# vandenheuvel/relp

Measured on AMD Instinct MI355X. Metric: simplex pivots/sec + wall-clock to optimal, Netlib 25fv47 @1 GPU, higher is better.
Workload: dtype f64; 1 GPU; Netlib 25FV47 821x1876, steepest-edge pricing, explicit-inverse carry, exact certificate inside the timed step, no presolve (+520 virtual artificials); carry=explicit, refactors=0, parallelism=1 LP per GPU x1, certified=True, objective_bits=1791

## Files before the change

### relp_amd/csrc/kernels.hip

```cpp
#include <hip/hip_runtime.h>
#include <hip/hip_ext.h>

#include <cmath>
#include <cstdlib>
#include <string>
#include <utility>

#include "kernels.hpp"
#include "pivot_step.hpp"
#include "price_step.hpp"
#include "solver.hpp"
#include "wave_ops.hpp"

namespace relp {


__global__ void budget_kernel(Ctl* ctl, long long add) {
    if (ctl->status == ST_BUDGET) ctl->status = ST_RUNNING;
    ctl->budget = ctl->iters + add;
}

typedef double f64x2_t __attribute__((ext_vector_type(2)));
template <int RULE, bool USE_LDS, int LPC, bool UNIT = false>
__global__ void __launch_bounds__(256) price_kernel(DeviceLP lp, int skip_weights, double tol_dual, int col_first,
                                                    int col_last, int cand_offset) {
    static_assert(!UNIT || LPC == 2, "generated columns are incidence columns");
    extern __shared__ __attribute__((aligned(16))) double smem[];
    __shared__ Cand s_cand[8];
    static_assert(LPC == ELL_W || LPC == 2, "one lane per padded entry (width 2 when no column has more than two entries: graph LPs)");
    constexpr int CPB = 256 / LPC;
    Ctl* ctl = lp.ctl;
    const int m = lp.m;
    const int g = threadIdx.x / LPC, sub = threadIdx.x % LPC;
    const int status = ctl->status;
    const int pending = (RULE == RELP_PIVOT_STEEPEST_EDGE) ? (ctl->pending && !skip_weights) : 0;
    const double gamma_q = ctl->gamma_q;
    const double alpha_pq = ctl->alpha_pq;
    const int leaving = ctl->leaving;
    const int last = ctl->last_selected;
    int base = col_first + blockIdx.x * CPB;
    int a = 0, b = 0, r0 = 0;
    double v0 = 0.0, cost_j = 0.0, g_j = 1.0;
    bool nonbasic = false;
    double sgn_j = 1.0;
    auto load_column = [&](int j) {
        a = b = r0 = 0;
        v0 = cost_j = 0.0;
        g_j = 1.0;
        nonbasic = false;
        sgn_j = 1.0;
        if (j < col_last) {
            const int pos_j = lp.pos[j];
            nonbasic = column_priced(pos_j);
            sgn_j = column_sign(pos_j);
            if (LPC != 2) {
                a = lp.col_start[j];
                b = lp.col_start[j + 1];
            }
            if (UNIT) {
                const unsigned code = (unsigned)lp.ell_rows[(size_t)j * LPC + sub];
                const bool absent = code == 0x7fffffffu;
                r0 = absent ? 0 : (int)(code & 0x7fffffffu);
                v0 = absent ? 0.0 : ((code >> 31) ? -1.0 : 1.0);
                cost_j = (double)lp.cost8[j];
            } else {
                r0 = lp.ell_rows[(size_t)j * LPC + sub];
                v0 = lp.ell_vals[(size_t)j * LPC + sub];
                cost_j = lp.cost[j];
            }
            if (RULE == RELP_PIVOT_STEEPEST_EDGE && !UNIT) g_j = lp.gamma[j];
        }
    };
    load_column(base + g);
    const double* v_pi = lp.minus_pi;
    const double* v_rho = lp.rho;
    const double* v_w = lp.w;
    if (USE_LDS) {
        double* s_pi = smem;
        double* s_rho = smem + m;
        double* s_w = smem + 2 * m;
        for (int i0 = threadIdx.x; i0 < m; i0 += 4 * 256) {
            double t_pi[4], t_rho[4], t_w[4];
#pragma unroll
            for (int u = 0; u < 4; ++u) {
                const int i = i0 + u * 256;
                t_pi[u] = i < m ? lp.minus_pi[i] : 0.0;
                t_rho[u] = i < m ? lp.rho[i] : 0.0;
                t_w[u] = i < m ? lp.w[i] : 0.0;
            }
#pragma unroll
            for (int u = 0; u < 4; ++u) {
                const int i = i0 + u * 256;
                if (i < m) {
                    s_pi[i] = t_pi[u];
                    s_rho[i] = t_rho[u];
                    s_w[i] = t_w[u];
                }
            }
        }
        v_pi = s_pi;
        v_rho = s_rho;
        v_w = s_w;
    }
    if (status != ST_RUNNING) return;
    if (USE_LDS) __syncthreads();

    Cand best = no_candidate();
    double best_cbar = 0.0;
    int best_row = 0, best_len = 0;
    double best_val = 0.0;
    while (base < col_last) {
        const int j = base + g;
        if (!nonbasic) { b = a; v0 = 0.0; }
        double d_pi, d_rho = 0.0, d_w = 0.0;
        if (UNIT) {
            d_pi = v0 * lp.minus_pi[r0];
            if (pending) {
                int hit = lp.rho_nz[r0] != 0 && v0 != 0.0;
                hit |= __shfl_xor(hit, 1);
                if (hit) {
                    d_rho = v0 * lp.rho[r0];
                    d_w = v0 * lp.w[r0];
                }
            }
        } else if (LPC == 2) {
            const double* t = lp.prw + (size_t)4 * r0;
            if (pending) {
                const f64x2_t lo = *reinterpret_cast<const f64x2_t*>(t);
                d_w = v0 * t[2];
                d_pi = v0 * lo.x;
                d_rho = v0 * lo.y;
            } else {
                d_pi = v0 * t[0];
            }
        } else {
            d_pi = v0 * v_pi[r0];
            if (pending) {
                d_rho = v0 * v_rho[r0];
                d_w = v0 * v_w[r0];
            }
        }
        for (int e = a + LPC + sub; e < b; e += LPC) {
            const int r = lp.row_index[e];
            const double v = lp.value[e];
            d_pi += v * v_pi[r];
            if (pending) {
                d_rho += v * v_rho[r];
                d_w += v * v_w[r];
            }
        }
        d_pi += dpp_f64<DPP_QUAD_1032, 0xF>(0.0, d_pi);
        if (LPC > 2) {
            d_pi += dpp_f64<DPP_QUAD_2301, 0xF>(0.0, d_pi);
            d_pi += dpp_f64<DPP_ROW_HALF_MIRROR, 0xF>(0.0, d_pi);
        }
        if (RULE == RELP_PIVOT_STEEPEST_EDGE) {
            d_rho += dpp_f64<DPP_QUAD_1032, 0xF>(0.0, d_rho);
            d_w += dpp_f64<DPP_QUAD_1032, 0xF>(0.0, d_w);
            if (LPC > 2) {
                d_rho += dpp_f64<DPP_QUAD_2301, 0xF>(0.0, d_rho);
                d_rho += dpp_f64<DPP_ROW_HALF_MIRROR, 0xF>(0.0, d_rho);
                d_w += dpp_f64<DPP_QUAD_2301, 0xF>(0.0, d_w);
                d_w += dpp_f64<DPP_ROW_HALF_MIRROR, 0xF>(0.0, d_w);
            }
        }
        int improved = 0;
        const double cbar = sgn_j * (cost_j + d_pi);
        const bool weight_changes = RULE == RELP_PIVOT_STEEPEST_EDGE && pending && (!UNIT || j == leaving || d_rho != 0.0);
        if (sub == 0 && nonbasic && (!UNIT || weight_changes || cbar < -tol_dual)) {
            double gam = g_j;
            if (UNIT && RULE == RELP_PIVOT_STEEPEST_EDGE) gam = lp.gamma[j];
            if (weight_changes) lp.gamma[j] = gam = weight_after_pivot(gam, d_rho, d_w, gamma_q, alpha_pq, j == leaving);
            bool candidate;
            const double key = price_key<RULE>(cbar, tol_dual, gam, j, last, lp.n, candidate);
            if (candidate && offer_candidate<RULE>(best, key, j)) {
                best_cbar = cbar;
                improved = 1;
            }
        }
        improved = __shfl(improved, threadIdx.x & (WAVE - 1) & ~(LPC - 1));
        if (improved) {
            best_row = r0;
            best_val = v0;
            best_len = LPC == 2 ? 2 : b - a;
        }
        base += gridDim.x * CPB;
        if (base < col_last) load_column(base + g);
    }
    const Cand blk = block_best_candidate<RULE>(best, s_cand);
    const int slot = cand_offset + blockIdx.x;
    int winner = (sub == 0 && blk.idx >= 0 && blk.idx == best.idx) ? 1 : 0;
    if (winner) publish_candidate(lp, slot, blk.key, blk.idx, best_cbar, best_len);
    winner = __shfl(winner, threadIdx.x & (WAVE - 1) & ~(LPC - 1));
    if (winner) publish_entry(lp, slot, sub, best_row, best_val);
    if (blk.idx < 0 && threadIdx.x == 0) publish_no_candidate(lp, slot);
}

template <int RULE>
__global__ void __launch_bounds__(256) price_unit_kernel(DeviceLP lp, int skip_weights, double tol_dual, int col_first,
                                                         int col_last, int cand_offset) {
    constexpr int U = PRICE_UNIT_ARCS;
    extern __shared__ __attribute__((aligned(16))) unsigned s_rho_bits[];
    __shared__ Cand s_cand[8];
    Ctl* ctl = lp.ctl;
#ifdef RELP_STAMPS
    unsigned long long t_prev__ = wall_clock64();
    const int stamp_base__ = blockIdx.x == 0 ? 32 : (blockIdx.x == gridDim.x - 1 ? 40 : -1);
    if (threadIdx.x == 0 && blockIdx.x == 0) {
        lp.dbg[48] += 1;
        *(volatile unsigned long long*)(lp.dbg + 49) = t_prev__;
    }
#define USTAMP(k) do { asm volatile("s_waitcnt vmcnt(0) lgkmcnt(0)" ::: "memory"); if (threadIdx.x == 0 && stamp_base__ >= 0) { unsigned long long t__ = wall_clock64(); lp.dbg[stamp_base__ + (k)] += t__ - t_prev__; t_prev__ = t__; } } while (0)
#else
#define USTAMP(k) do {} while (0)
#endif
    const int status = ctl->status;
    const int pending = (RULE == RELP_PIVOT_STEEPEST_EDGE) ? (ctl->pending && !skip_weights) : 0;
    const double gamma_q = ctl->gamma_q;
    const double alpha_pq = ctl->alpha_pq;
    const int leaving = ctl->leaving;
    const int last = ctl->last_selected;
    const uint2* arcs = reinterpret_cast<const uint2*>(lp.ell_rows);
    unsigned ca[U], cb[U];
    int pos[U];
    double cost[U];
    auto load_arcs = [&](int base) {
#pragma unroll
        for (int u = 0; u < U; ++u) {
            const int j = base + u * 256 + threadIdx.x;
            ca[u] = cb[u] = 0x7fffffffu;
            pos[u] = 0;
            cost[u] = 0.0;
            if (j < col_last) {
                const uint2 c = arcs[j];
                ca[u] = c.x;
                cb[u] = c.y;
                pos[u] = lp.pos[j];
                cost[u] = (double)lp.cost8[j];
            }
        }
// ... 1475 lines not shown
    __shared__ double s_amount;
    if (threadIdx.x == 0) {
        const double cbar_q = ctl->cbar_q;
        int toggle = -1;
        double amount = 0.0;
        if (p < 0 && !flip) {
            ctl_unbounded(*ctl, q, 0);
        } else if (flip) {
            const double sgn_q = lp.flipped[q] ? -1.0 : 1.0;
            toggle = q;
            amount = ub_q * sgn_q;
            ctl_bound_flip(lp, *ctl, q, sgn_q, ub_q, cbar_q, ctl->minus_obj, ctl->iters);
            ctl->xp = ub_q;
        } else {
            const int leaving_flipped = bounded ? lp.flipped[leaving] : 0;
            if (step.leaves_at_upper) {
                toggle = leaving;
                amount = up_p * (leaving_flipped ? -1.0 : 1.0);
            }
            lp.basis[p] = q;
            push_touched(lp, *ctl, p);
            ctl_basis_change(lp, *ctl, bounded, q, p, leaving, leaving_flipped, step, ub_q, cbar_q, alpha_pq, ctl->gamma_q, total, ctl->minus_obj, ctl->iters);
            ctl->rho_buf ^= 1;
        }
        s_toggle = toggle;
        s_amount = amount;
    }
    __syncthreads();
    const int toggle = s_toggle;
    if (toggle >= 0) {
        const double amount = s_amount;
        for (int e = lp.col_start[toggle] + threadIdx.x; e < lp.col_start[toggle + 1]; e += blockDim.x)
            lp.rhs[lp.row_index[e]] -= amount * lp.value[e];
    }
}

constexpr int K2F_NW = K2F_THREADS / WAVE;
constexpr int K2F_INLINE_BLOCKS = 128;

struct K2fShared {
    double akey[K2F_NW];
    unsigned long long arank[K2F_NW];
    double red[K2F_NW + 2];
    double red2[K2F_NW + 2];
    double cbarv[K2F_MAX_BLOCKS];
    int crows[K2F_INLINE_BLOCKS * ELL_W];
    double cvals[K2F_INLINE_BLOCKS * ELL_W];
    int clen[K2F_INLINE_BLOCKS];
    int rows[K2_COL_CHUNK];
    double vals[K2_COL_CHUNK];
    double bcast[4];
    int ibcast[2];
};
template <int RULE>
__device__ __forceinline__ void k2f_candidates(const DeviceLP& lp, int n_price_blocks, K2fShared& sm, double& ckey, unsigned long long& crank) {
    const int tid = threadIdx.x;
    for (int b = tid; b < n_price_blocks; b += K2F_THREADS) {
        const int j = lp.cand_j[b];
        const double k = lp.cand_key[b];
        sm.cbarv[b] = lp.cand_cbar[b];
        offer_entering<RULE>(k, j, b, ckey, crank);
    }
    if (n_price_blocks <= K2F_INLINE_BLOCKS) {
        for (int e = tid; e < n_price_blocks * ELL_W; e += K2F_THREADS) {
            sm.crows[e] = lp.cand_rows[e];
            sm.cvals[e] = lp.cand_vals[e];
        }
        for (int b = tid; b < n_price_blocks; b += K2F_THREADS) sm.clen[b] = lp.cand_len[b];
    }
}
template <int RULE>
__device__ __forceinline__ int k2f_entering(double ckey, unsigned long long crank, K2fShared& sm, double& cbar_q, int& winner_block) {
    const int q = entering_winner<RULE>(ckey, crank, sm.akey, sm.arank, winner_block);
    cbar_q = q >= 0 ? sm.cbarv[winner_block] : 0.0;
    return q;
}
template <int R>
__device__ __forceinline__ void k2f_ftran_inline(const DeviceLP& lp, const double* T, const K2fShared& sm, int q, int winner_block,
                                                 double (&al)[R], int& ca, int& cb_) {
    const int tid = threadIdx.x, m = lp.m, ld = lp.ld;
    const int len = sm.clen[winner_block];
#pragma unroll
    for (int r = 0; r < R; ++r) {
        const int i = tid + r * K2F_THREADS;
        if (i >= m || len < 0) continue;
        const double* col = T + i;
        double t[ELL_W];
#pragma unroll
        for (int e = 0; e < ELL_W; ++e) t[e] = col[(size_t)sm.crows[winner_block * ELL_W + e] * ld];
        double a0 = 0.0;
#pragma unroll
        for (int e = 0; e < ELL_W; ++e) a0 += t[e] * sm.cvals[winner_block * ELL_W + e];
        al[r] = a0;
    }
    if (len > ELL_W || len < 0) {
        ca = lp.col_start[q] + (len < 0 ? 0 : ELL_W);
        cb_ = lp.col_start[q + 1];
    }
}
template <int R>
__device__ __forceinline__ void k2f_ftran_csc(const DeviceLP& lp, const double* T, K2fShared& sm, int ca, int cb_, double (&al)[R]) {
    const int tid = threadIdx.x, m = lp.m, ld = lp.ld;
    for (int c0 = ca; c0 < cb_; c0 += K2_COL_CHUNK) {
        const int cnt = min(K2_COL_CHUNK, cb_ - c0);
        __syncthreads();
        for (int e = tid; e < cnt; e += K2F_THREADS) {
            sm.rows[e] = lp.row_index[c0 + e];
            sm.vals[e] = lp.value[c0 + e];
        }
        __syncthreads();
        if constexpr (R <= 8) {
            double acc[R][4];
            int row[R];
#pragma unroll
            for (int r = 0; r < R; ++r) {
                const int i = tid + r * K2F_THREADS;
                row[r] = i < m ? i : 0;
                acc[r][0] = acc[r][1] = acc[r][2] = acc[r][3] = 0.0;
            }
            int e = 0;
            for (; e + 4 <= cnt; e += 4) {
                const size_t o0 = (size_t)sm.rows[e] * ld, o1 = (size_t)sm.rows[e + 1] * ld, o2 = (size_t)sm.rows[e + 2] * ld, o3 = (size_t)sm.rows[e + 3] * ld;
                const double v0 = sm.vals[e], v1 = sm.vals[e + 1], v2 = sm.vals[e + 2], v3 = sm.vals[e + 3];
                double x[R][4];
#pragma unroll
                for (int r = 0; r < R; ++r) {
                    x[r][0] = T[o0 + row[r]];
                    x[r][1] = T[o1 + row[r]];
                    x[r][2] = T[o2 + row[r]];
                    x[r][3] = T[o3 + row[r]];
                }
#pragma unroll
                for (int r = 0; r < R; ++r) {
                    acc[r][0] += x[r][0] * v0;
                    acc[r][1] += x[r][1] * v1;
                    acc[r][2] += x[r][2] * v2;
                    acc[r][3] += x[r][3] * v3;
                }
            }
            for (; e < cnt; ++e) {
                const size_t o = (size_t)sm.rows[e] * ld;
                const double v = sm.vals[e];
                double x[R];
#pragma unroll
                for (int r = 0; r < R; ++r) x[r] = T[o + row[r]];
#pragma unroll
// ... 50 lines not shown
    __syncthreads();
    if (wave == 0) {
        double t1 = lane < K2F_NW ? sm.red[lane] : 0.0;
        double t2 = lane < K2F_NW ? sm.red2[lane] : INFINITY;
        t1 = wave_sum(t1);
        t2 = wave_min(t2);
        if (lane == LAST) {
            sm.red[K2F_NW] = t1;
            sm.red2[K2F_NW] = t2;
        }
    }
    __syncthreads();
    gamma_q = 1.0 + sm.red[K2F_NW];
    theta_max = sm.red2[K2F_NW];
}
template <int R>
__device__ __forceinline__ int k2f_pass2(bool textbook, const double (&al)[R], const bool (&eligible)[R], const double (&room)[R],
                                         const int (&bas)[R], double theta_max, K2fShared& sm) {
    double hkey = 0.0;
    unsigned long long hrank = RANK_NONE;
#pragma unroll
    for (int r = 0; r < R; ++r) {
        const double mag = fabs(al[r]);
        if (eligible[r] && harris_accepts(room[r], mag, theta_max))
            keep_better(harris_key(textbook, mag), leaving_rank(bas[r], threadIdx.x + r * K2F_THREADS), hkey, hrank);
    }
    block_argbest(hkey, hrank, sm.akey, sm.arank);
    return leaving_row(hrank);
}
template <int R>
__device__ __forceinline__ void k2f_broadcast_row(int p, const double (&al)[R], const double (&xb)[R], const double (&room)[R],
                                                  const int (&bas)[R], K2fShared& sm) {
#pragma unroll
    for (int r = 0; r < R; ++r) {
        if ((int)threadIdx.x + r * K2F_THREADS == p) {
            sm.bcast[1] = al[r];
            sm.bcast[2] = xb[r];
            sm.bcast[3] = room[r];
            sm.ibcast[0] = bas[r];
        }
    }
    __syncthreads();
}

template <int RULE, int R>
__global__ void __launch_bounds__(K2F_THREADS) ftran_ratio_fast_kernel(DeviceLP lp, int n_price_blocks, double tol_pivot,
                                                                     double harris_delta, int skip_artificial_rows,
                                                                     int mode, int n_alpha_slices) {
    __shared__ K2fShared sm;
    Ctl* ctl = lp.ctl;
    STAMP_INIT;
    const int tid = threadIdx.x;
    const int m = lp.m;
    const int status = ctl->status;
    const long long iters = ctl->iters;
    const long long budget = ctl->budget;
    const int forced_q = ctl->forced_q;
    const int forced_p = ctl->forced_p;
    const double minus_obj = ctl->minus_obj;
    double xb[R];
    int bas[R];
#pragma unroll
    for (int r = 0; r < R; ++r) {
        const int i = tid + r * K2F_THREADS;
        xb[r] = i < m ? lp.xB[i] : 0.0;
        bas[r] = i < m ? lp.basis[i] : 0x7fffffff;
    }
    double ckey = 0.0;
    unsigned long long crank = RANK_NONE;
    const bool preselected = n_alpha_slices > 0;
    const int q_pre = preselected ? ctl->q : -1;
    const double cbar_pre = preselected ? ctl->cbar_q : 0.0;
    double ain[R];
#pragma unroll
    for (int r = 0; r < R; ++r) {
        const int i = tid + r * K2F_THREADS;
        ain[r] = (preselected && i < m) ? lp.alpha_in[i] : 0.0;
    }
    if (!preselected) k2f_candidates<RULE>(lp, n_price_blocks, sm, ckey, crank);
    const bool inline_column = forced_q < 0 && !preselected && n_price_blocks <= K2F_INLINE_BLOCKS;
    if (status != ST_RUNNING) return;
    STAMP(0);
    if (mode == 0 && iters >= budget) {
        if (tid == 0) ctl_budget(*ctl);
        return;
    }
    int q;
    double cbar_q;
    int winner_block = 0;
    if (preselected && forced_q < 0) {
        q = q_pre;
        cbar_q = cbar_pre;
    } else if (forced_q < 0) {
        q = k2f_entering<RULE>(ckey, crank, sm, cbar_q, winner_block);
    } else {
        q = forced_q;
        if (tid == 0) {
            double cb = lp.cost[forced_q];
            for (int e = lp.col_start[forced_q]; e < lp.col_start[forced_q + 1]; ++e) cb += lp.value[e] * lp.minus_pi[lp.row_index[e]];
            sm.bcast[0] = cb;
        }
        __syncthreads();
        cbar_q = sm.bcast[0];
        __syncthreads();
    }
    STAMP(1);
    if (q < 0) {
        if (tid == 0) ctl_no_entering(*ctl, mode);
        return;
    }
    if (mode == 1) {
        if (tid == 0) ctl_entering_only(*ctl, q, cbar_q);
        return;
    }
    double al[R];
#pragma unroll
    for (int r = 0; r < R; ++r) al[r] = 0.0;
    int ca = 0, cb_ = 0;
    if (inline_column) {
        k2f_ftran_inline<R>(lp, lp.Binv, sm, q, winner_block, al, ca, cb_);
    } else if (!preselected) {
        ca = lp.col_start[q];
        cb_ = lp.col_start[q + 1];
    }
    if (preselected) {
#pragma unroll
        for (int r = 0; r < R; ++r) al[r] += ain[r];
    }
    k2f_ftran_csc<R>(lp, lp.Binv, sm, ca, cb_, al);
    STAMP(2);
    const bool bounded = lp.ub != nullptr;
    double sgn_q = 1.0, ub_q = INFINITY;
// ... 102 lines not shown
        }
    }
    STAMP(5);
    const int leaving_flipped = bounded ? lp.flipped[leaving] : 0;
    if (step.leaves_at_upper) {
        const double sgn_l = leaving_flipped ? -1.0 : 1.0;
        for (int e = lp.col_start[leaving] + tid; e < lp.col_start[leaving + 1]; e += K2F_THREADS)
            lp.rhs[lp.row_index[e]] -= step.ub_leaving * sgn_l * lp.value[e];
    }
    if (bounded) __syncthreads();
    if (tid == 0) {
        lp.basis[p] = q;
        push_touched(lp, *ctl, p);
        if (lp.eta_cap > 0) {
            int is_new = 0;
            if (eta_slot_p < 0) {
                const int k = ctl->eta_count;
                lp.eta_slot[p] = k;
                lp.eta_rows[k] = p;
                ctl->eta_count = k + 1;
                is_new = 1;
            }
            ctl->eta_new = is_new;
            ctl->eta_version = ctl->eta_version + 1;
        }
        ctl_basis_change(lp, *ctl, bounded, q, p, leaving, leaving_flipped, step, ub_q, cbar_q, alpha_pq, gamma_q, total, minus_obj, iters);
        ctl->rho_buf ^= 1;
    }
    STAMP(6);
}

constexpr int KF_THREADS = K2F_THREADS;
constexpr int KF_NW = KF_THREADS / WAVE;
template <int RULE, int KF_R>
__global__ void __launch_bounds__(KF_THREADS) pivot_fused_kernel(DeviceLP lp, DeviceLP::State in, DeviceLP::State out, int n_price_blocks,
                                                                 double tol_pivot, double harris_delta, int skip_artificial_rows) {
    constexpr int R = KF_R;
    constexpr int KF_U = KF_R * KF_THREADS / WAVE;
    constexpr int KF_M = KF_R * KF_THREADS;
    __shared__ K2fShared sm;
    __shared__ double s_alpha[KF_M];
    const Ctl* ctl = in.ctl;
    const int tid = threadIdx.x;
    const int lane = tid & (WAVE - 1), wave = tid / WAVE;
#ifdef RELP_STAMPS
    unsigned long long t_prev__ = clock64();
    if (tid == 0 && blockIdx.x == 0) lp.dbg[63] += 1;
#define FSTAMP(k) do { if (tid == 0 && blockIdx.x == 0) { unsigned long long t__ = clock64(); lp.dbg[(k)] += t__ - t_prev__; t_prev__ = t__; } } while (0)
#else
#define FSTAMP(k) do {} while (0)
#endif
    const int m = lp.m, ld = lp.ld;
    const bool writer = blockIdx.x == 0;
    const int status = ctl->status;
    const long long iters = ctl->iters;
    const long long budget = ctl->budget;
    const double minus_obj = ctl->minus_obj;
    const int t_buf = ctl->t_buf;
    double xb[R];
    int bas[R];
#pragma unroll
    for (int r = 0; r < R; ++r) {
        const int i = tid + r * KF_THREADS;
        xb[r] = i < m ? in.xB[i] : 0.0;
        bas[r] = i < m ? in.basis[i] : 0x7fffffff;
    }
    double ckey = 0.0;
    unsigned long long crank = RANK_NONE;
    k2f_candidates<RULE>(lp, n_price_blocks, sm, ckey, crank);
    const bool inline_column = n_price_blocks <= K2F_INLINE_BLOCKS;
    auto hand_on = [&](auto verdict) {
        if (!writer) return;
#pragma unroll
        for (int r = 0; r < R; ++r) {
            const int i = tid + r * KF_THREADS;
            if (i < m) {
                out.xB[i] = xb[r];
                out.basis[i] = bas[r];
            }
        }
        if (tid == 0) {
            Ctl c = *ctl;
            verdict(c);
            c.forced_q = -1;
            c.forced_p = -1;
            *out.ctl = c;
        }
    };
    if (status != ST_RUNNING) {
        hand_on([](Ctl&) {});
        return;
    }
    FSTAMP(0);
    if (iters >= budget) {
        hand_on([](Ctl& c) { ctl_budget(c); });
        return;
    }
    double cbar_q;
    int winner_block = 0;
    const int q = k2f_entering<RULE>(ckey, crank, sm, cbar_q, winner_block);
    if (q < 0) {
        hand_on([](Ctl& c) { ctl_no_entering(c, 0); });
        return;
    }
    FSTAMP(1);
    const int j_own = blockIdx.x * KF_NW + wave;
    const bool own = j_own < m;
    const double* t_old = (t_buf ? lp.Binv2 : lp.Binv);
    double* t_new = (t_buf ? lp.Binv : lp.Binv2);
    const double* c_old = t_old + (size_t)(own ? j_own : 0) * ld;
    double o[KF_U];
#pragma unroll
    for (int u = 0; u < KF_U; ++u) {
        const int i = lane + u * WAVE;
        o[u] = (own && i < m) ? c_old[i] : 0.0;
    }
    const double pi_old = (own && lane == LAST) ? lp.minus_pi[j_own] : 0.0;
    double al[R];
#pragma unroll
    for (int r = 0; r < R; ++r) al[r] = 0.0;
    int ca = 0, cb_ = 0;
    if (inline_column) {
        k2f_ftran_inline<R>(lp, t_old, sm, q, winner_block, al, ca, cb_);
    } else {
        ca = lp.col_start[q];
        cb_ = lp.col_start[q + 1];
    }
    k2f_ftran_csc<R>(lp, t_old, sm, ca, cb_, al);
    FSTAMP(2);
    const HarrisRule harris = harris_rule(harris_delta);
    double sumsq = 0.0, theta = INFINITY;
    bool eligible[R];
    double room[R];
    k2f_pass1<R>(lp, false, al, xb, bas, tol_pivot, harris.slack, skip_artificial_rows, eligible, room, sumsq, theta);
#pragma unroll
    for (int r = 0; r < R; ++r) s_alpha[tid + r * KF_THREADS] = al[r];
    double gamma_q, theta_max;
    k2f_reduce(sm, sumsq, theta, gamma_q, theta_max);
    FSTAMP(3);
    const int p = k2f_pass2<R>(harris.textbook, al, eligible, room, bas, theta_max, sm);
    if (p < 0) {
        hand_on([q](Ctl& c) { ctl_unbounded(c, q, 0); });
        return;
    }
    FSTAMP(4);
    k2f_broadcast_row<R>(p, al, xb, room, bas, sm);
    const double alpha_pq = sm.bcast[1];
    const int leaving = sm.ibcast[0];
    const Step step = step_decision(false, false, p, alpha_pq, sm.bcast[2], sm.bcast[3], INFINITY);
    const double xp = step.xp;
    if (writer) {
#pragma unroll
        for (int r = 0; r < R; ++r) {
            const int i = tid + r * KF_THREADS;
            if (i < m) {
                lp.alpha[i] = al[r];
                out.xB[i] = (i == p) ? xp : xb[r] - al[r] * xp;
                out.basis[i] = (i == p) ? q : bas[r];
            }
        }
        if (tid == 0) {
            Ctl c = *ctl;
            ctl_basis_change(lp, c, false, q, p, leaving, 0, step, INFINITY, cbar_q, alpha_pq, gamma_q, 0, minus_obj, iters);
            c.t_buf = t_buf ^ 1;
            *out.ctl = c;
        }
    }
    FSTAMP(5);
    if (!own) return;
    const int u_p = p >> 6, lane_p = p & (WAVE - 1);
    double o_p = 0.0;
#pragma unroll
    for (int u = 0; u < KF_U; ++u) o_p = (u == u_p) ? o[u] : o_p;
    const double r_j = __shfl(o_p, lane_p) / alpha_pq;
    double* c_new = t_new + (size_t)j_own * ld;
    double w_j = 0.0;
#pragma unroll
    for (int u = 0; u < KF_U; ++u) {
        const int i = lane + u * WAVE;
        const double a = s_alpha[i];
        w_j += a * o[u];
        if (i < m) c_new[i] = (i == p) ? r_j : ((a != 0.0) ? o[u] - a * r_j : o[u]);
    }
    w_j = wave_sum(w_j);
    if (lane == LAST) {
        lp.w[j_own] = w_j;
        lp.rho[j_own] = r_j;
        lp.minus_pi[j_own] = pi_old - cbar_q * r_j;
    }
    FSTAMP(6);
}
#undef FSTAMP
__global__ void __launch_bounds__(256) begin_batch_kernel(DeviceLP lp, long long add) {
    const DeviceLP::State s0 = lp.state[0];
    for (int i = threadIdx.x; i < lp.m; i += 256) {
        s0.xB[i] = lp.xB[i];
        s0.basis[i] = lp.basis[i];
    }
    if (threadIdx.x == 0) {
        Ctl c = *lp.ctl;
        if (c.status == ST_BUDGET) c.status = ST_RUNNING;
        c.budget = c.iters + add;
        *lp.ctl = c;
        *s0.ctl = c;
    }
}
__global__ void __launch_bounds__(256) commit_kernel(DeviceLP lp, int parity) {
    const DeviceLP::State last = lp.state[parity];
    const int t_buf = last.ctl->t_buf;
    const int m = lp.m, ld = lp.ld;
    if (t_buf) {
        const int lane = threadIdx.x & (WAVE - 1);
        for (int j = blockIdx.x * 4 + threadIdx.x / WAVE; j < m; j += gridDim.x * 4) {
            const double* src = lp.Binv2 + (size_t)j * ld;
            double* dst = lp.Binv + (size_t)j * ld;
            for (int i = lane; i < m; i += WAVE) dst[i] = src[i];
        }
    }
    if (blockIdx.x == 0) {
        for (int i = threadIdx.x; i < m; i += 256) {
            lp.xB[i] = last.xB[i];
            lp.basis[i] = last.basis[i];
        }
        if (threadIdx.x == 0) {
            Ctl c = *last.ctl;
            c.t_buf = 0;
            *lp.ctl = c;
            if (lp.ctl_mirror) {
                *lp.ctl_mirror = c;
                __threadfence_system();
            }
        }
    }
// ... 830 lines not shown
```

### relp_amd/csrc/solver.hpp

```cpp
#pragma once
#include <cstdlib>
#include <cstring>
#include <cstddef>
#include <hip/hip_runtime.h>

#include <atomic>
#include <memory>
#include <mutex>
#include <stdexcept>
#include <string>
#include <vector>

#include "../../include/relp_amd.h"
#include "device_columns.hpp"
#include "kernel_path.hpp"
#include "device_memory.hpp"
#include "model.hpp"
#include "lu.hpp"

namespace relp {

struct ExactPrimal;
struct ExactWitnesses;
struct CertifyScratch {
// ... 3 lines not shown
        void* ptr;
        size_t bytes;
        bool busy;
    };
    std::vector<Block> blocks;
    std::vector<Block> pinned;
    void* take_pinned(size_t bytes);
    void give_back_pinned(void* ptr);
    int digit_hints[2] = {0, 0};
    std::shared_ptr<const void> statics;
    void* take(size_t bytes);
    void give_back(void* ptr);
    void release();
};
std::vector<std::pair<int, std::string>> exact_primal_values(const ExactPrimal& primal);
std::shared_ptr<const ExactPrimal> make_exact_primal(const std::vector<int>& columns, const std::vector<Rat>& values);
int exact_witness_mode(const ExactWitnesses& witnesses);
std::vector<std::pair<int, std::string>> exact_witness_values(const ExactWitnesses& witnesses, int which);
void certify_basis(const StandardForm& form, const std::vector<int>& basis_provider_columns, int device, hipStream_t stream,
                   std::string* objective, bool* certified, long long* repair_pivots, std::string* message, int mode, int entering,
                   std::shared_ptr<const ExactPrimal>* primal, CertifyScratch* scratch,
                   std::shared_ptr<const ExactWitnesses>* witnesses = nullptr);

struct Ctl {
    int status;
    int q;
    int p;
    int leaving;
    int pending;
    int forced_q;
    int forced_p;
    int last_selected;
    long long iters;
    long long budget;
    double cbar_q;
    double alpha_pq;
    double gamma_q;
    double xp;
    double minus_obj;
    double residual;
    double scan_value;
    int scan_column;
    int nz_count;
    int eta_count;
    int touched_count;
    double flip_cost;
    long long bound_flips;
    int k2_forced;
    int t_buf;
    int eta_version;
    int eta_new;
    int rho_buf;
};

enum : int { ST_RUNNING = 0, ST_NO_ENTERING = 1, ST_UNBOUNDED = 2, ST_BUDGET = 3, ST_REFACTOR = 4, ST_REFACTOR_FAILED = 5 };

struct DeviceLP {
    int m = 0, n = 0, n_art = 0, ld = 0;
    int n_dense = 0, dense_first = 0, dense_ld = 0;
    double* dense_val = nullptr;
    signed char* dense_val8 = nullptr;
    int dense_full = 0, dense_csc_start = 0;
    int dense_lane = 0;
    float* dense_val32 = nullptr;
    double* alpha_part = nullptr;
    double* alpha_in = nullptr;
    int eta_cap = 0;
    double* eta_cols = nullptr;
    int* eta_rows = nullptr;
    int* eta_slot = nullptr;
    double* eta_gather = nullptr;
    double* eta_dot_part = nullptr;
    int* slack_of_row = nullptr;
    int track_touched = 0;
    int* touched = nullptr;
    int* tlist = nullptr;
    int* col_start = nullptr;
    int* row_index = nullptr;
    double* value = nullptr;
    int* row_start = nullptr;
    int* col_index = nullptr;
    double* row_value = nullptr;
    double* cost = nullptr;
    double* cost1 = nullptr;
    double* cost2 = nullptr;
    double* rhs = nullptr;
    double* xB = nullptr;
    double* minus_pi = nullptr;
    int* basis = nullptr;
    int* pos = nullptr;
    double* gamma = nullptr;
    double* cb = nullptr;
    int* cb_idx = nullptr;
    double* Binv = nullptr;
    double* Binv2 = nullptr;
    double* R = nullptr;
    double* alpha = nullptr;
    double* rho = nullptr;
    double* w = nullptr;
    int* nz_index = nullptr;
    double* nz_alpha = nullptr;
    double* cand_key = nullptr;
    int* cand_j = nullptr;
    double* cand_cbar = nullptr;
    int* cand_rows = nullptr;
    double* cand_vals = nullptr;
// ... 304 lines not shown
```

### relp_amd/csrc/wave_ops.hpp

```cpp
#pragma once
#include <hip/hip_runtime.h>
#include <cmath>
#include "solver.hpp"

namespace relp {

#ifdef RELP_STAMPS
#define STAMP(k) do { if (threadIdx.x == 0) { unsigned long long t__ = clock64(); lp.dbg[(k)] += t__ - t_prev__; t_prev__ = t__; } } while (0)
#define STAMP_INIT unsigned long long t_prev__ = clock64(); if (threadIdx.x == 0) lp.dbg[63] += 1
#else
#define STAMP(k) do {} while (0)
#define STAMP_INIT do {} while (0)
#endif

struct Cand {
    double key;
    int idx;
    int aux;
};

enum : int { TIE_LARGER_IDX = 0, TIE_SMALLER_IDX = 1, TIE_SMALLER_AUX = 2 };

template <int TIE>
__device__ __forceinline__ Cand better(Cand a, Cand b) {
    bool take_b;
    if (TIE == TIE_LARGER_IDX) take_b = (b.key > a.key) | ((b.key == a.key) & (b.idx > a.idx));
    else if (TIE == TIE_SMALLER_IDX) take_b = (b.key > a.key) | ((b.key == a.key) & (b.idx < a.idx));
    else take_b = (b.key > a.key) | ((b.key == a.key) & ((b.aux < a.aux) | ((b.aux == a.aux) & (b.idx < a.idx))));
    take_b = (a.idx < 0) | ((b.idx >= 0) & take_b);
    Cand r;
    r.key = take_b ? b.key : a.key;
    r.idx = take_b ? b.idx : a.idx;
    r.aux = take_b ? b.aux : a.aux;
    return r;
}

constexpr int DPP_QUAD_1032 = 0xB1;
constexpr int DPP_QUAD_2301 = 0x4E;
constexpr int DPP_ROW_HALF_MIRROR = 0x141;
constexpr int DPP_ROW_ROR4 = 0x124;
constexpr int DPP_ROW_ROR8 = 0x128;
constexpr int DPP_ROW_BCAST15 = 0x142;
constexpr int DPP_ROW_BCAST31 = 0x143;

template <int CTRL, int ROW_MASK>
__device__ __forceinline__ int dpp_i32(int old, int v) {
    return __builtin_amdgcn_update_dpp(old, v, CTRL, ROW_MASK, 0xF, false);
}
template <int CTRL, int ROW_MASK>
__device__ __forceinline__ double dpp_f64(double old, double v) {
    const int lo = dpp_i32<CTRL, ROW_MASK>(__double2loint(old), __double2loint(v));
    const int hi = dpp_i32<CTRL, ROW_MASK>(__double2hiint(old), __double2hiint(v));
    return __hiloint2double(hi, lo);
}
template <int CTRL, int ROW_MASK>
__device__ __forceinline__ Cand dpp_cand(Cand v) {
    Cand o;
    o.key = dpp_f64<CTRL, ROW_MASK>(v.key, v.key);
    o.idx = dpp_i32<CTRL, ROW_MASK>(v.idx, v.idx);
    o.aux = dpp_i32<CTRL, ROW_MASK>(v.aux, v.aux);
    return o;
}

template <int CTRL, int ROW_MASK> __device__ __forceinline__ double dpp_move(double old, double v) { return dpp_f64<CTRL, ROW_MASK>(old, v); }
template <int CTRL, int ROW_MASK> __device__ __forceinline__ int dpp_move(int old, int v) { return dpp_i32<CTRL, ROW_MASK>(old, v); }
template <int CTRL, int ROW_MASK> __device__ __forceinline__ Cand dpp_move(Cand, Cand v) { return dpp_cand<CTRL, ROW_MASK>(v); }
// ... 122 lines not shown
```

Baseline: 56440 pivots/s.

## Hoist and batch global loads ahead of dependent work in price and pivot kernels

Restructures the price kernel to issue next-column loads, including up to two extra CSC entries, before the LDS staging, so their latency overlaps other work. The fused pivot kernels issue xB, basis, candidate and old-inverse-column loads at kernel entry, before reading control state and choosing the entering column, and clamp indices in place of predicating the loads. It adds compiler scheduling barriers and a field-wise Ctl copy to keep the loads grouped. The cost is higher register pressure and some redundant clamped loads.

```diff
diff --git a/relp_amd/csrc/kernels.hip b/relp_amd/csrc/kernels.hip
--- a/relp_amd/csrc/kernels.hip
+++ b/relp_amd/csrc/kernels.hip
@@ -32,46 +32,84 @@
     Ctl* ctl = lp.ctl;
     const int m = lp.m;
     const int g = threadIdx.x / LPC, sub = threadIdx.x % LPC;
+    int base = col_first + blockIdx.x * CPB;
+    int a = 0, b = 0, r0 = 0;
+    double v0 = 0.0, cost_j = 0.0, g_j = 1.0;
+    bool nonbasic = false;
+    double sgn_j = 1.0;
+    bool in_n = false, has1_n = false, has2_n = false;
+    int pos_n = 0, a_n = 0, b_n = 0, r0_n = 0, cost8_n = 0;
+    double v0_n = 0.0, cost_n = 0.0, g_n = 1.0;
+    int xr1_n = 0, xr2_n = 0;
+    double xv1_n = 0.0, xv2_n = 0.0;
+    bool has1 = false, has2 = false;
+    int xr1 = 0, xr2 = 0;
+    double xv1 = 0.0, xv2 = 0.0;
+    auto issue_column = [&](int j) {
+        in_n = j < col_last;
+        const int jc = in_n ? j : max(col_last - 1, 0);
+        pos_n = lp.pos[jc];
+        if (LPC != 2) {
+            a_n = lp.col_start[jc];
+            b_n = lp.col_start[jc + 1];
+        }
+        r0_n = lp.ell_rows[(size_t)jc * LPC + sub];
+        if (UNIT) {
+            cost8_n = lp.cost8[jc];
+        } else {
+            v0_n = lp.ell_vals[(size_t)jc * LPC + sub];
+            cost_n = lp.cost[jc];
+        }
+        if (RULE == RELP_PIVOT_STEEPEST_EDGE && !UNIT) g_n = lp.gamma[jc];
+    };
+    auto issue_extension = [&]() {
+        if constexpr (LPC == ELL_W) {
+            const bool priced = in_n && column_priced(pos_n);
+            const int e1 = a_n + LPC + sub, e2 = a_n + 2 * LPC + sub;
+            has1_n = priced && e1 < b_n;
+            has2_n = priced && e2 < b_n;
+            if (has1_n) {
+                xr1_n = lp.row_index[e1];
+                xv1_n = lp.value[e1];
+            }
+            if (has2_n) {
+                xr2_n = lp.row_index[e2];
+                xv2_n = lp.value[e2];
+            }
+        }
+    };
+    auto accept_column = [&]() {
+        nonbasic = in_n && column_priced(pos_n);
+        sgn_j = in_n ? column_sign(pos_n) : 1.0;
+        a = in_n ? a_n : 0;
+        b = in_n ? b_n : 0;
+        if (UNIT) {
+            const unsigned code = (unsigned)r0_n;
+            const bool absent = !in_n || code == 0x7fffffffu;
+            r0 = absent ? 0 : (int)(code & 0x7fffffffu);
+            v0 = absent ? 0.0 : ((code >> 31) ? -1.0 : 1.0);
+            cost_j = in_n ? (double)cost8_n : 0.0;
+        } else {
+            r0 = in_n ? r0_n : 0;
+            v0 = in_n ? v0_n : 0.0;
+            cost_j = in_n ? cost_n : 0.0;
+        }
+        g_j = (RULE == RELP_PIVOT_STEEPEST_EDGE && !UNIT && in_n) ? g_n : 1.0;
+        has1 = has1_n;
+        has2 = has2_n;
+        xr1 = xr1_n;
+        xv1 = xv1_n;
+        xr2 = xr2_n;
+        xv2 = xv2_n;
+    };
     const int status = ctl->status;
     const int pending = (RULE == RELP_PIVOT_STEEPEST_EDGE) ? (ctl->pending && !skip_weights) : 0;
     const double gamma_q = ctl->gamma_q;
     const double alpha_pq = ctl->alpha_pq;
     const int leaving = ctl->leaving;
     const int last = ctl->last_selected;
-    int base = col_first + blockIdx.x * CPB;
-    int a = 0, b = 0, r0 = 0;
-    double v0 = 0.0, cost_j = 0.0, g_j = 1.0;
-    bool nonbasic = false;
-    double sgn_j = 1.0;
-    auto load_column = [&](int j) {
-        a = b = r0 = 0;
-        v0 = cost_j = 0.0;
-        g_j = 1.0;
-        nonbasic = false;
-        sgn_j = 1.0;
-        if (j < col_last) {
-            const int pos_j = lp.pos[j];
-            nonbasic = column_priced(pos_j);
-            sgn_j = column_sign(pos_j);
-            if (LPC != 2) {
-                a = lp.col_start[j];
-                b = lp.col_start[j + 1];
-            }
-            if (UNIT) {
-                const unsigned code = (unsigned)lp.ell_rows[(size_t)j * LPC + sub];
-                const bool absent = code == 0x7fffffffu;
-                r0 = absent ? 0 : (int)(code & 0x7fffffffu);
-                v0 = absent ? 0.0 : ((code >> 31) ? -1.0 : 1.0);
-                cost_j = (double)lp.cost8[j];
-            } else {
-                r0 = lp.ell_rows[(size_t)j * LPC + sub];
-                v0 = lp.ell_vals[(size_t)j * LPC + sub];
-                cost_j = lp.cost[j];
-            }
-            if (RULE == RELP_PIVOT_STEEPEST_EDGE && !UNIT) g_j = lp.gamma[j];
-        }
-    };
-    load_column(base + g);
+    RELP_LOADS_PINNED();
+    issue_column(base + g);
     const double* v_pi = lp.minus_pi;
     const double* v_rho = lp.rho;
     const double* v_w = lp.w;
@@ -79,8 +117,27 @@
         double* s_pi = smem;
         double* s_rho = smem + m;
         double* s_w = smem + 2 * m;
-        for (int i0 = threadIdx.x; i0 < m; i0 += 4 * 256) {
-            double t_pi[4], t_rho[4], t_w[4];
+        double t_pi[4], t_rho[4], t_w[4];
+#pragma unroll
+        for (int u = 0; u < 4; ++u) {
+            const int i = threadIdx.x + u * 256;
+            const int ic = i < m ? i : 0;
+            t_pi[u] = lp.minus_pi[ic];
+            t_rho[u] = lp.rho[ic];
+            t_w[u] = lp.w[ic];
+        }
+        issue_extension();
+        RELP_LOADS_ISSUED();
+#pragma unroll
+        for (int u = 0; u < 4; ++u) {
+            const int i = threadIdx.x + u * 256;
+            if (i < m) {
+                s_pi[i] = t_pi[u];
+                s_rho[i] = t_rho[u];
+                s_w[i] = t_w[u];
+            }
+        }
+        for (int i0 = threadIdx.x + 4 * 256; i0 < m; i0 += 4 * 256) {
 #pragma unroll
             for (int u = 0; u < 4; ++u) {
                 const int i = i0 + u * 256;
@@ -101,7 +158,11 @@
         v_pi = s_pi;
         v_rho = s_rho;
         v_w = s_w;
-    }
+    } else {
+        issue_extension();
+        RELP_LOADS_ISSUED();
+    }
+    accept_column();
     if (status != ST_RUNNING) return;
     if (USE_LDS) __syncthreads();
 
@@ -140,7 +201,23 @@
                 d_w = v0 * v_w[r0];
             }
         }
-        for (int e = a + LPC + sub; e < b; e += LPC) {
+        if constexpr (LPC == ELL_W) {
+            if (has1) {
+                d_pi += xv1 * v_pi[xr1];
+                if (pending) {
+                    d_rho += xv1 * v_rho[xr1];
+                    d_w += xv1 * v_w[xr1];
+                }
+            }
+            if (has2) {
+                d_pi += xv2 * v_pi[xr2];
+                if (pending) {
+                    d_rho += xv2 * v_rho[xr2];
+                    d_w += xv2 * v_w[xr2];
+                }
+            }
+        }
+        for (int e = a + 3 * LPC + sub; e < b; e += LPC) {
             const int r = lp.row_index[e];
             const double v = lp.value[e];
             d_pi += v * v_pi[r];
@@ -185,7 +262,13 @@
             best_len = LPC == 2 ? 2 : b - a;
         }
         base += gridDim.x * CPB;
-        if (base < col_last) load_column(base + g);
+        if (base < col_last) {
+            issue_column(base + g);
+            RELP_LOADS_ISSUED();
+            issue_extension();
+            RELP_LOADS_ISSUED();
+            accept_column();
+        }
     }
     const Cand blk = block_best_candidate<RULE>(best, s_cand);
     const int slot = cand_offset + blockIdx.x;
@@ -1767,21 +1850,54 @@
     double bcast[4];
     int ibcast[2];
 };
+static_assert(K2F_INLINE_BLOCKS * ELL_W <= 2 * K2F_THREADS, "the inline entries are two loads per thread");
+struct K2fCandidateLoads {
+    int j, len;
+    double key, cbar;
+    int row[2];
+    double val[2];
+};
+__device__ __forceinline__ void k2f_candidates_issue(const DeviceLP& lp, int n_price_blocks, K2fCandidateLoads& c) {
+    const int tid = threadIdx.x;
+    const int bc = tid < n_price_blocks ? tid : 0;
+    c.j = lp.cand_j[bc];
+    c.key = lp.cand_key[bc];
+    c.cbar = lp.cand_cbar[bc];
+    c.len = lp.cand_len[bc];
+#pragma unroll
+    for (int t = 0; t < 2; ++t) {
+        const int e = tid + t * K2F_THREADS;
+        const int ec = e < n_price_blocks * ELL_W ? e : 0;
+        c.row[t] = lp.cand_rows[ec];
+        c.val[t] = lp.cand_vals[ec];
+    }
+}
 template <int RULE>
-__device__ __forceinline__ void k2f_candidates(const DeviceLP& lp, int n_price_blocks, K2fShared& sm, double& ckey, unsigned long long& crank) {
+__device__ __forceinline__ void k2f_candidates_fold(const DeviceLP& lp, int n_price_blocks, K2fShared& sm, const K2fCandidateLoads& c,
+                                                    double& ckey, unsigned long long& crank) {
     const int tid = threadIdx.x;
-    for (int b = tid; b < n_price_blocks; b += K2F_THREADS) {
+    if (tid < n_price_blocks) {
+        sm.cbarv[tid] = c.cbar;
+        offer_entering<RULE>(c.key, c.j, tid, ckey, crank);
+    }
+    if (n_price_blocks <= K2F_INLINE_BLOCKS) {
+#pragma unroll
+        for (int t = 0; t < 2; ++t) {
+            const int e = tid + t * K2F_THREADS;
+            if (e < n_price_blocks * ELL_W) {
+                sm.crows[e] = c.row[t];
+                sm.cvals[e] = c.val[t];
+            }
+        }
+        if (tid < n_price_blocks) sm.clen[tid] = c.len;
+    }
+    for (int b = tid + K2F_THREADS; b < n_price_blocks; b += K2F_THREADS) {
         const int j = lp.cand_j[b];
         const double k = lp.cand_key[b];
-        sm.cbarv[b] = lp.cand_cbar[b];
+        const double cb = lp.cand_cbar[b];
+        RELP_LOADS_ISSUED();
+        sm.cbarv[b] = cb;
         offer_entering<RULE>(k, j, b, ckey, crank);
-    }
-    if (n_price_blocks <= K2F_INLINE_BLOCKS) {
-        for (int e = tid; e < n_price_blocks * ELL_W; e += K2F_THREADS) {
-            sm.crows[e] = lp.cand_rows[e];
-            sm.cvals[e] = lp.cand_vals[e];
-        }
-        for (int b = tid; b < n_price_blocks; b += K2F_THREADS) sm.clen[b] = lp.cand_len[b];
     }
 }
 template <int RULE>
@@ -1795,18 +1911,27 @@
                                                  double (&al)[R], int& ca, int& cb_) {
     const int tid = threadIdx.x, m = lp.m, ld = lp.ld;
     const int len = sm.clen[winner_block];
-#pragma unroll
-    for (int r = 0; r < R; ++r) {
-        const int i = tid + r * K2F_THREADS;
-        if (i >= m || len < 0) continue;
-        const double* col = T + i;
-        double t[ELL_W];
-#pragma unroll
-        for (int e = 0; e < ELL_W; ++e) t[e] = col[(size_t)sm.crows[winner_block * ELL_W + e] * ld];
-        double a0 = 0.0;
-#pragma unroll
-        for (int e = 0; e < ELL_W; ++e) a0 += t[e] * sm.cvals[winner_block * ELL_W + e];
-        al[r] = a0;
+    if (len >= 0) {
+        constexpr int G = R <= 4 ? R : 4;
+#pragma unroll
+        for (int rg = 0; rg < R; rg += G) {
+            double t[G][ELL_W];
+#pragma unroll
+            for (int g = 0; g < G; ++g) {
+                const int i = tid + (rg + g) * K2F_THREADS;
+                const double* col = T + (i < m ? i : 0);
+#pragma unroll
+                for (int e = 0; e < ELL_W; ++e) t[g][e] = col[(size_t)sm.crows[winner_block * ELL_W + e] * ld];
+            }
+            RELP_LOADS_ISSUED();
+#pragma unroll
+            for (int g = 0; g < G; ++g) {
+                double a0 = 0.0;
+#pragma unroll
+                for (int e = 0; e < ELL_W; ++e) a0 += t[g][e] * sm.cvals[winner_block * ELL_W + e];
+                if (tid + (rg + g) * K2F_THREADS < m) al[rg + g] = a0;
+            }
+        }
     }
     if (len > ELL_W || len < 0) {
         ca = lp.col_start[q] + (len < 0 ? 0 : ELL_W);
@@ -1963,32 +2088,46 @@
     STAMP_INIT;
     const int tid = threadIdx.x;
     const int m = lp.m;
+    kernel_args_ready(ctl, lp.xB, lp.basis, lp.alpha_in, lp.cand_j, lp.cand_key, lp.cand_cbar, lp.cand_len, lp.cand_rows, lp.cand_vals, m, n_price_blocks,
+                      n_alpha_slices);
+    double xb[R];
+    int bas[R];
+    double ain[R];
+    const bool preselected = n_alpha_slices > 0;
+    const double* ain_from = preselected ? lp.alpha_in : lp.xB;
+#pragma unroll
+    for (int r = 0; r < R; ++r) {
+        const int i = tid + r * K2F_THREADS;
+        const int ic = i < m ? i : 0;
+        xb[r] = lp.xB[ic];
+        bas[r] = lp.basis[ic];
+        ain[r] = ain_from[ic];
+    }
+    double ckey = 0.0;
+    unsigned long long crank = RANK_NONE;
+    K2fCandidateLoads cand;
+    k2f_candidates_issue(lp, n_price_blocks, cand);
+    RELP_LOADS_PINNED();
     const int status = ctl->status;
     const long long iters = ctl->iters;
     const long long budget = ctl->budget;
     const int forced_q = ctl->forced_q;
     const int forced_p = ctl->forced_p;
     const double minus_obj = ctl->minus_obj;
-    double xb[R];
-    int bas[R];
+    const int q_loaded = ctl->q;
+    const double cbar_loaded = ctl->cbar_q;
+    RELP_LOADS_ISSUED();
+    const int q_pre = preselected ? q_loaded : -1;
+    const double cbar_pre = preselected ? cbar_loaded : 0.0;
 #pragma unroll
     for (int r = 0; r < R; ++r) {
-        const int i = tid + r * K2F_THREADS;
-        xb[r] = i < m ? lp.xB[i] : 0.0;
-        bas[r] = i < m ? lp.basis[i] : 0x7fffffff;
-    }
-    double ckey = 0.0;
-    unsigned long long crank = RANK_NONE;
-    const bool preselected = n_alpha_slices > 0;
-    const int q_pre = preselected ? ctl->q : -1;
-    const double cbar_pre = preselected ? ctl->cbar_q : 0.0;
-    double ain[R];
-#pragma unroll
-    for (int r = 0; r < R; ++r) {
-        const int i = tid + r * K2F_THREADS;
-        ain[r] = (preselected && i < m) ? lp.alpha_in[i] : 0.0;
-    }
-    if (!preselected) k2f_candidates<RULE>(lp, n_price_blocks, sm, ckey, crank);
+        if (tid + r * K2F_THREADS >= m) {
+            xb[r] = 0.0;
+            bas[r] = 0x7fffffff;
+        }
+        if (!preselected || tid + r * K2F_THREADS >= m) ain[r] = 0.0;
+    }
+    if (!preselected) k2f_candidates_fold<RULE>(lp, n_price_blocks, sm, cand, ckey, crank);
     const bool inline_column = forced_q < 0 && !preselected && n_price_blocks <= K2F_INLINE_BLOCKS;
     if (status != ST_RUNNING) return;
     STAMP(0);
@@ -2197,22 +2336,35 @@
 #endif
     const int m = lp.m, ld = lp.ld;
     const bool writer = blockIdx.x == 0;
+    kernel_args_ready(ctl, in.xB, in.basis, lp.cand_j, lp.cand_key, lp.cand_cbar, lp.cand_len, lp.cand_rows, lp.cand_vals, m, n_price_blocks);
+    double xb[R];
+    int bas[R];
+#pragma unroll
+    for (int r = 0; r < R; ++r) {
+        const int i = tid + r * KF_THREADS;
+        const int ic = i < m ? i : 0;
+        xb[r] = in.xB[ic];
+        bas[r] = in.basis[ic];
+    }
+    double ckey = 0.0;
+    unsigned long long crank = RANK_NONE;
+    K2fCandidateLoads cand;
+    k2f_candidates_issue(lp, n_price_blocks, cand);
+    RELP_LOADS_PINNED();
     const int status = ctl->status;
     const long long iters = ctl->iters;
     const long long budget = ctl->budget;
     const double minus_obj = ctl->minus_obj;
     const int t_buf = ctl->t_buf;
-    double xb[R];
-    int bas[R];
+    RELP_LOADS_ISSUED();
 #pragma unroll
     for (int r = 0; r < R; ++r) {
-        const int i = tid + r * KF_THREADS;
-        xb[r] = i < m ? in.xB[i] : 0.0;
-        bas[r] = i < m ? in.basis[i] : 0x7fffffff;
-    }
-    double ckey = 0.0;
-    unsigned long long crank = RANK_NONE;
-    k2f_candidates<RULE>(lp, n_price_blocks, sm, ckey, crank);
+        if (tid + r * KF_THREADS >= m) {
+            xb[r] = 0.0;
+            bas[r] = 0x7fffffff;
+        }
+    }
+    k2f_candidates_fold<RULE>(lp, n_price_blocks, sm, cand, ckey, crank);
     const bool inline_column = n_price_blocks <= K2F_INLINE_BLOCKS;
     auto hand_on = [&](auto verdict) {
         if (!writer) return;
@@ -2225,11 +2377,12 @@
             }
         }
         if (tid == 0) {
-            Ctl c = *ctl;
+            Ctl c;
+            ctl_copy(c, *ctl);
             verdict(c);
             c.forced_q = -1;
             c.forced_p = -1;
-            *out.ctl = c;
+            ctl_copy(*out.ctl, c);
         }
     };
     if (status != ST_RUNNING) {
@@ -2241,6 +2394,19 @@
         hand_on([](Ctl& c) { ctl_budget(c); });
         return;
     }
+    const int j_own = blockIdx.x * KF_NW + wave;
+    const bool own = j_own < m;
+    const double* t_old = (t_buf ? lp.Binv2 : lp.Binv);
+    double* t_new = (t_buf ? lp.Binv : lp.Binv2);
+    const double* c_old = t_old + (size_t)(own ? j_own : 0) * ld;
+    double o[KF_U];
+#pragma unroll
+    for (int u = 0; u < KF_U; ++u) {
+        const int i = lane + u * WAVE;
+        o[u] = c_old[i < m ? i : 0];
+    }
+    double pi_old = lp.minus_pi[own ? j_own : 0];
+    RELP_LOADS_PINNED();
     double cbar_q;
     int winner_block = 0;
     const int q = k2f_entering<RULE>(ckey, crank, sm, cbar_q, winner_block);
@@ -2249,18 +2415,6 @@
         return;
     }
     FSTAMP(1);
-    const int j_own = blockIdx.x * KF_NW + wave;
-    const bool own = j_own < m;
-    const double* t_old = (t_buf ? lp.Binv2 : lp.Binv);
-    double* t_new = (t_buf ? lp.Binv : lp.Binv2);
-    const double* c_old = t_old + (size_t)(own ? j_own : 0) * ld;
-    double o[KF_U];
-#pragma unroll
-    for (int u = 0; u < KF_U; ++u) {
-        const int i = lane + u * WAVE;
-        o[u] = (own && i < m) ? c_old[i] : 0.0;
-    }
-    const double pi_old = (own && lane == LAST) ? lp.minus_pi[j_own] : 0.0;
     double al[R];
 #pragma unroll
     for (int r = 0; r < R; ++r) al[r] = 0.0;
@@ -2271,6 +2425,11 @@
         ca = lp.col_start[q];
         cb_ = lp.col_start[q + 1];
     }
+#pragma unroll
+    for (int u = 0; u < KF_U; ++u) {
+        if (!own || lane + u * WAVE >= m) o[u] = 0.0;
+    }
+    if (!own || lane != LAST) pi_old = 0.0;
     k2f_ftran_csc<R>(lp, t_old, sm, ca, cb_, al);
     FSTAMP(2);
     const HarrisRule harris = harris_rule(harris_delta);
@@ -2305,10 +2464,11 @@
             }
         }
         if (tid == 0) {
-            Ctl c = *ctl;
+            Ctl c;
+            ctl_copy(c, *ctl);
             ctl_basis_change(lp, c, false, q, p, leaving, 0, step, INFINITY, cbar_q, alpha_pq, gamma_q, 0, minus_obj, iters);
             c.t_buf = t_buf ^ 1;
-            *out.ctl = c;
+            ctl_copy(*out.ctl, c);
         }
     }
     FSTAMP(5);
@@ -2320,10 +2480,14 @@
     const double r_j = __shfl(o_p, lane_p) / alpha_pq;
     double* c_new = t_new + (size_t)j_own * ld;
     double w_j = 0.0;
+    double a_u[KF_U];
+#pragma unroll
+    for (int u = 0; u < KF_U; ++u) a_u[u] = s_alpha[lane + u * WAVE];
+    __builtin_amdgcn_sched_barrier(0);
 #pragma unroll
     for (int u = 0; u < KF_U; ++u) {
         const int i = lane + u * WAVE;
-        const double a = s_alpha[i];
+        const double a = a_u[u];
         w_j += a * o[u];
         if (i < m) c_new[i] = (i == p) ? r_j : ((a != 0.0) ? o[u] - a * r_j : o[u]);
     }
diff --git a/relp_amd/csrc/solver.hpp b/relp_amd/csrc/solver.hpp
--- a/relp_amd/csrc/solver.hpp
+++ b/relp_amd/csrc/solver.hpp
@@ -79,6 +79,18 @@
     int eta_new;
     int rho_buf;
 };
+
+#if defined(__HIPCC__)
+#define RELP_CTL_FIELDS(X) X(status) X(q) X(p) X(leaving) X(pending) X(forced_q) X(forced_p) X(last_selected) X(iters) X(budget) X(cbar_q) \
+    X(alpha_pq) X(gamma_q) X(xp) X(minus_obj) X(residual) X(scan_value) X(scan_column) X(nz_count) X(eta_count) X(touched_count) \
+    X(flip_cost) X(bound_flips) X(k2_forced) X(t_buf) X(eta_version) X(eta_new) X(rho_buf)
+__device__ __forceinline__ void ctl_copy(Ctl& dst, const Ctl& src) {
+    static_assert(sizeof(Ctl) == 8 * 4 + 2 * 8 + 7 * 8 + 4 * 4 + 2 * 8 + 5 * 4 + 4, "a field of Ctl is missing from RELP_CTL_FIELDS");
+#define RELP_CTL_COPY(f) dst.f = src.f;
+    RELP_CTL_FIELDS(RELP_CTL_COPY)
+#undef RELP_CTL_COPY
+}
+#endif
 
 enum : int { ST_RUNNING = 0, ST_NO_ENTERING = 1, ST_UNBOUNDED = 2, ST_BUDGET = 3, ST_REFACTOR = 4, ST_REFACTOR_FAILED = 5 };
 
diff --git a/relp_amd/csrc/wave_ops.hpp b/relp_amd/csrc/wave_ops.hpp
--- a/relp_amd/csrc/wave_ops.hpp
+++ b/relp_amd/csrc/wave_ops.hpp
@@ -12,6 +12,13 @@
 #define STAMP(k) do {} while (0)
 #define STAMP_INIT do {} while (0)
 #endif
+
+template <class A>
+__device__ __forceinline__ void kernel_arg_ready(A a) { asm volatile("" ::"s"(a)); }
+template <class... A>
+__device__ __forceinline__ void kernel_args_ready(A... a) { (kernel_arg_ready(a), ...); }
+#define RELP_LOADS_PINNED() asm volatile("" ::: "memory")
+#define RELP_LOADS_ISSUED() do { asm volatile("" ::: "memory"); __builtin_amdgcn_sched_barrier(0); } while (0)
 
 struct Cand {
     double key;
```

Result: faster. 58260 pivots/s (median of 6 runs) (+3.2%).
